# Qualcomm-AI-research/transformer-quantization

Measured on AMD Instinct MI355X. Metric: M elems/sec fake-quant fwd (BERT-base act tensor); achieved HBM GB/s vs peak, higher is better.
Workload: dtype f32; 1 GPU; BERT-base W8A8 per-tensor asym 8-bit activation fake-quant, running-minmax calibrated, fixed-range fwd, hidden [1024,512,768] bf16 per GPU (BASELINE configs[1]); storage_dtype=bf16, parallelism=dp1 (independent shards, no data-path collective)

## Files before the change

transformer-quantization_amd/csrc_py/tq_fastcall.c:

```c
#define PY_SSIZE_T_CLEAN
#include <Python.h>
#include <stdint.h>

typedef int (*fq_fwd_t)(const void*, void*, void*, int, uint64_t, int, const void*, void*);

static int as_u64(PyObject* o, uint64_t* out) {
  if (o == Py_None) { *out = 0; return 0; }
  unsigned long long v = PyLong_AsUnsignedLongLong(o);
  if (v == (unsigned long long)-1 && PyErr_Occurred()) return -1;
  *out = (uint64_t)v;
  return 0;
}

static PyObject* fake_quant_fwd(PyObject* self, PyObject* const* args, Py_ssize_t nargs) {
  (void)self;
  if (nargs != 9) {
    PyErr_SetString(PyExc_TypeError, "fake_quant_fwd(fn, x, y, idx, idx_dtype, n, dtype, q, stream)");
    return NULL;
  }
  uint64_t v[9];
  for (int i = 0; i < 9; ++i)
    if (as_u64(args[i], &v[i])) return NULL;
  if (v[0] == 0) {
    PyErr_SetString(PyExc_ValueError, "fake_quant_fwd: NULL entry point");
    return NULL;
  }
  fq_fwd_t fn = (fq_fwd_t)(uintptr_t)v[0];
  int rc = fn((const void*)(uintptr_t)v[1], (void*)(uintptr_t)v[2], (void*)(uintptr_t)v[3], (int)v[4], v[5], (int)v[6],
              (const void*)(uintptr_t)v[7], (void*)(uintptr_t)v[8]);
  return PyLong_FromLong(rc);
}

typedef int (*calib_tensor_t)(const void*, uint64_t, int, int, const float*, const float*, float*, float*, double, int, int,
                              float, int, float*, float*, uint8_t*, void*, void*, size_t, uint32_t*, void*);

static PyObject* calibrate_tensor(PyObject* self, PyObject* const* args, Py_ssize_t nargs) {
  (void)self;
  if (nargs != 22) {
    PyErr_SetString(PyExc_TypeError, "calibrate_tensor(fn, <the 21 arguments of tq_calibrate_tensor>)");
    return NULL;
  }
  uint64_t v[22];
  double momentum = 0.0, eps = 0.0;
  for (int i = 0; i < 22; ++i) {
    if (i == 9 || i == 12) {
      const double d = PyFloat_AsDouble(args[i]);
      if (d == -1.0 && PyErr_Occurred()) return NULL;
      if (i == 9) momentum = d; else eps = d;
      v[i] = 0;
    } else if (as_u64(args[i], &v[i])) {
      return NULL;
    }
  }
  if (v[0] == 0) {
    PyErr_SetString(PyExc_ValueError, "calibrate_tensor: NULL entry point");
    return NULL;
  }
  calib_tensor_t fn = (calib_tensor_t)(uintptr_t)v[0];
#define P(i) ((void*)(uintptr_t)v[i])
  int rc = fn(P(1), v[2], (int)v[3], (int)v[4], (const float*)P(5), (const float*)P(6), (float*)P(7), (float*)P(8), momentum,
              (int)v[10], (int)v[11], (float)eps, (int)v[13], (float*)P(14), (float*)P(15), (uint8_t*)P(16), P(17), P(18),
              (size_t)v[19], (uint32_t*)P(20), P(21));
#undef P
  return PyLong_FromLong(rc);
}

typedef int (*ptr12_t)(uintptr_t, uintptr_t, uintptr_t, uintptr_t, uintptr_t, uintptr_t, uintptr_t, uintptr_t, uintptr_t,
                       uintptr_t, uintptr_t, uintptr_t);

static PyObject* call_ptrs(PyObject* self, PyObject* const* args, Py_ssize_t nargs) {
  (void)self;
  if (nargs < 1 || nargs > 13) {
    PyErr_SetString(PyExc_TypeError, "call_ptrs(fn, up to 12 integer / pointer arguments)");
    return NULL;
  }
  uint64_t v[13] = {0};
  for (Py_ssize_t i = 0; i < nargs; ++i)
    if (as_u64(args[i], &v[i])) return NULL;
  if (v[0] == 0) {
    PyErr_SetString(PyExc_ValueError, "call_ptrs: NULL entry point");
    return NULL;
  }
  int rc = ((ptr12_t)(uintptr_t)v[0])(v[1], v[2], v[3], v[4], v[5], v[6], v[7], v[8], v[9], v[10], v[11], v[12]);
  return PyLong_FromLong(rc);
}

static PyMethodDef methods[] = {
    {"fake_quant_fwd", (PyCFunction)(void (*)(void))fake_quant_fwd, METH_FASTCALL, "tq_fake_quant_fwd through a raw address"},
    {"calibrate_tensor", (PyCFunction)(void (*)(void))calibrate_tensor, METH_FASTCALL, "tq_calibrate_tensor through a raw address"},
    {"call_ptrs", (PyCFunction)(void (*)(void))call_ptrs, METH_FASTCALL, "int f(uintptr_t...) through a raw address"},
    {NULL, NULL, 0, NULL}};

static struct PyModuleDef moddef = {PyModuleDef_HEAD_INIT, "_tq_fastcall", "fast foreign calls into libtq_hip.so", -1, methods,
                                    NULL, NULL, NULL, NULL};

PyMODINIT_FUNC PyInit__tq_fastcall(void) { return PyModule_Create(&moddef); }
```

transformer-quantization_amd/quantization/_hip.py:

```python
import ctypes as C
import os

import torch

_HERE = os.path.dirname(os.path.abspath(__file__))
LIB_PATH = os.environ.get('TQ_LIB_PATH') or os.path.join(os.path.dirname(_HERE), 'lib', 'libtq_hip.so')

TQ_F32, TQ_BF16, TQ_F16 = 0, 1, 2
IDX_NONE, IDX_F32, IDX_I8, IDX_U8, IDX_I16, IDX_I32, IDX_I8_M128 = range(7)
ACT_NONE, ACT_RELU, ACT_GELU, ACT_TANH = range(4)
EST_CURRENT, EST_ALL, EST_RUNNING = 0, 1, 2
ADA_SIGMOID, ADA_HARD_SIGMOID, ADA_SIGMOID_TEMP = 0, 1, 2

_DTYPES = {torch.float32: TQ_F32, torch.bfloat16: TQ_BF16, torch.float16: TQ_F16}
_IDX_DTYPES = {torch.float32: IDX_F32, torch.int8: IDX_I8, torch.uint8: IDX_U8,
               torch.int16: IDX_I16, torch.int32: IDX_I32}


class TQError(RuntimeError):
    pass


class tq_quantizer(C.Structure):
    _fields_ = [('delta', C.c_void_p), ('zero_float', C.c_void_p), ('signed_flag', C.c_void_p),
# ... 130 lines not shown
    'tq_mse_candidates_grouped': (_int, [_vp, _u64, _u64, _u64, _int, _vp, _u64, _vp, _vp, _sz, _vp]),
    'tq_mse_ordered_workspace_bytes': (_sz, [_u64, _u64, _u64]),
    'tq_mse_candidates_ordered': (_int, [_vp, _u64, _u64, _int, _vp, _u64, _int, _vp, _vp, _vp, _sz, _vp]),
    'tq_xent_candidates': (_int, [_vp, _u64, _u64, _vp, _u64, _vp, _vp]),
    'tq_argmin_select': (_int, [_vp, _u64, _u64, _vp, _vp, _vp, _vp, _vp, _vp]),
    'tq_adaround_fwd': (_int, [_vp, _vp, _vp, _u64, _QP, _int, _int, _f, _vp]),
    'tq_adaround_init_alpha': (_int, [_vp, _vp, _u64, _QP, _int, _f, _vp]),
    'tq_adaround_bwd': (_int, [_vp, _vp, _vp, _vp, _u64, _QP, _int, _f, _vp]),
    'tq_adaround_bwd_adam_sched': (_int, [_vp, _vp, _vp, _vp, _vp, _u64, _QP, _int, _f, _vp, _f, _f, _f, _f, _vp]),
    'tq_adaround_bwd_adam': (_int, [_vp, _vp, _vp, _vp, _vp, _vp, _u64, _QP, _int, _f, _f, _f, _f,
                                    _f, _f, _f, _int, _vp]),
    'tq_adaround_reg': (_int, [_vp, _u64, _int, _f, _f, _f, _vp, _vp, _sz, _vp]),
    'tq_reduce_workspace_bytes': (_sz, [_u64]),
    'tq_recon_loss': (_int, [_vp, _vp, _u64, _u64, _u64, _vp, _vp, _sz, _vp]),
}

_lib = None


def load_library(path=None):
    global _lib
    if _lib is not None and path is None:
        return _lib
    p = path or LIB_PATH
    if not os.path.exists(p):
        raise TQError(
            f'{p} not found: build it with `python transformer-quantization_amd/build.py` '
            '(hipcc --offload-arch=gfx950).  There is no CPU fallback.')
    lib = C.CDLL(p)
    for name, (res, args) in SIGNATURES.items():
        fn = getattr(lib, name)
        fn.restype = res
        fn.argtypes = args
    if lib.tq_abi_version() != ABI_VERSION:
        raise TQError('libtq_hip.so ABI version mismatch: the library says %d, this binding is written for %d -- rebuild '
                      '(python transformer-quantization_amd/build.py)' % (lib.tq_abi_version(), ABI_VERSION))
    if path is None:
        _lib = lib
    return lib


_fastcall_mod, _fastcall_tried = None, False


def fastcall():
    global _fastcall_mod, _fastcall_tried
    if _fastcall_tried:
        return _fastcall_mod
    _fastcall_tried = True
    if os.environ.get('TQ_FASTCALL', '1') == '0':
        return None
    import glob
    import importlib.machinery
    import importlib.util
    for path in sorted(glob.glob(os.path.join(os.path.dirname(LIB_PATH), '_tq_fastcall*.so'))):
        try:
            loader = importlib.machinery.ExtensionFileLoader('_tq_fastcall', path)
            spec = importlib.util.spec_from_loader('_tq_fastcall', loader)
            mod = importlib.util.module_from_spec(spec)
            loader.exec_module(mod)
            _fastcall_mod = mod
            break
        except Exception:
            continue
    return _fastcall_mod


def entry_address(fn):
    return C.cast(fn, C.c_void_p).value


def _check(rc, lib):
    if rc != 0:
        raise TQError(f'libtq_hip: {lib.tq_last_error().decode()} (code {rc})')


def _ptr(t):
    return None if t is None else t.data_ptr()


_raw_stream = getattr(torch._C, '_cuda_getCurrentRawStream', None)


def _stream():
    if _raw_stream is not None:
        return _raw_stream(torch.cuda.current_device())
    return torch.cuda.current_stream().cuda_stream


def _need_device(t, what):
    if not t.is_cuda:
        raise TQError(f'{what}: tensor lives on {t.device}; the fake-quant path only runs on a '
                      'ROCm device (no CPU fallback)')


def _need_f32(what, *tensors):
    for t in tensors:
        if t is not None and t.dtype != torch.float32:
            raise TQError(f'{what}: fp32 tensors required, got {t.dtype} (call .float() on the layer first)')


def _dtype_code(t, what):
    try:
        return _DTYPES[t.dtype]
    except KeyError:
        hint = ' -- float64 (--double) runs the layered quantizer path only' if t.dtype == torch.float64 else ''
        raise TQError(f'{what}: dtype {t.dtype} not supported (fp32 / bf16 / fp16){hint}') from None


def _device_guarded(fn):
    import functools

    _Tensor, _cur = torch.Tensor, torch.cuda.current_device

    @functools.wraps(fn)
    def wrapper(self, *args, **kwargs):
        idx = -1
        for a in args:
            if isinstance(a, _Tensor):
                i = a.get_device()
                if i < 0:
                    continue
                if idx < 0:
                    idx = i
                elif i != idx:
                    raise TQError(f'{fn.__name__}: operands live on different devices (cuda:{idx} and cuda:{i})')
        if idx < 0:
            for a in args:
                if isinstance(a, (tuple, list)):
                    for b in a:
                        if isinstance(b, _Tensor) and b.get_device() >= 0:
                            idx = b.get_device()
                            break
                    if idx >= 0:
                        break
        if idx < 0 or idx == _cur():
            return fn(self, *args, **kwargs)
        with torch.cuda.device(idx):
            return fn(self, *args, **kwargs)
    return wrapper


class HipBackend:

    name = 'hip'

    def __init__(self):
        self.lib = load_library()
        self._ws = {}
        self._qdesc_cache = {}
        self._ws_bytes = {}
        self._counters = {}
        self._calib_tensor_addr = None

    def _workspace(self, device, nbytes):
        key = (device.index, _stream())
        ws = self._ws.get(key)
        if ws is None or ws.numel() < nbytes:
            ws = torch.empty(max(int(nbytes), 1 << 16), dtype=torch.uint8, device=device)
            self._ws[key] = ws
        return ws

    def _calib_ws_bytes(self, n, n_params, inner):
        key = (n, n_params, inner)
        v = self._ws_bytes.get(key)
        if v is None:
            if len(self._ws_bytes) > 4096:
                self._ws_bytes.clear()
            v = self._ws_bytes[key] = self.lib.tq_calibrate_workspace_bytes(n, n_params, inner)
        return v

    def to_device_f32(self, v, like=None):
        if torch.is_tensor(v):
            if v.is_cuda:
                return v if v.dtype == torch.float32 else v.float()
            dev = like.device if (like is not None and like.is_cuda) else torch.device(
                'cuda', torch.cuda.current_device())
            return v.detach().to(device=dev, dtype=torch.float32)
        dev = like.device if (like is not None and like.is_cuda) else torch.device(
            'cuda', torch.cuda.current_device())
        return torch.tensor(v, dtype=torch.float64).float().to(dev)

    def _qdesc(self, delta, zero_float, signed, n_bits, symmetric, log_domain, eps, n_params, inner):
        key = (None if delta is None else delta.data_ptr(), None if zero_float is None else zero_float.data_ptr(),
               None if signed is None else signed.data_ptr(), n_bits, symmetric, log_domain, eps, n_params, inner)
        cache = self._qdesc_cache
        d = cache.get(key)
        if d is None:
            if len(cache) > 8192:
                cache.clear()
            d = cache[key] = tq_quantizer(key[0], key[1], key[2], int(n_bits), int(bool(symmetric)),
                                          int(bool(log_domain)), float(eps), int(n_params), int(inner))
        return d

    @staticmethod
    def _as_f64(t, like):
        if t is None:
            return None
        t = t.detach()
        if t.dtype != torch.float64 or t.device != like.device:
            t = t.to(device=like.device, dtype=torch.float64)
        return t.contiguous()

    def _qdesc_f64(self, delta, zero_float, signed, n_bits, symmetric, log_domain, eps, n_params, inner):
        return tq_quantizer_f64(_ptr(delta), _ptr(zero_float), _ptr(signed), int(n_bits), int(bool(symmetric)),
                                int(bool(log_domain)), 0, float(eps), int(n_params), int(inner))

    def _fake_quant_f64(self, x, delta, zero_float, signed, n_bits, symmetric, log_domain, eps, n_params, inner,
                        want_y, want_idx):
        x = x.contiguous()
        d, z = self._as_f64(delta, x), self._as_f64(zero_float, x)
        y = torch.empty_like(x) if want_y else None
        idx = torch.empty_like(x) if want_idx else None
        q = self._qdesc_f64(d, z, signed, n_bits, symmetric, log_domain, eps, n_params, inner)
        rc = self.lib.tq_fake_quant_fwd_f64(_ptr(x), _ptr(y), _ptr(idx), x.numel(), C.byref(q), _stream())
        _check(rc, self.lib)
        return y, idx

    def fake_quant(self, x, delta, zero_float, signed, n_bits, symmetric, log_domain, eps,
                   n_params, inner, want_y=True, idx_dtype=None):
        _need_device(x, 'fake_quant')
        if x.dtype == torch.float64:
            if idx_dtype not in (None, torch.float32, torch.float64):
                raise TQError('fake_quant: float64 tensors emit float64 indices only')
            return self._fake_quant_f64(x, delta, zero_float, signed, n_bits, symmetric, log_domain, eps, n_params,
                                        inner, want_y, idx_dtype is not None)
        x = x.contiguous()
        y = torch.empty_like(x) if want_y else None
        idx = torch.empty(x.shape, dtype=idx_dtype, device=x.device) if idx_dtype is not None else None
        q = self._qdesc(delta, zero_float, signed, n_bits, symmetric, log_domain, eps, n_params, inner)
        rc = self.lib.tq_fake_quant_fwd(_ptr(x), _ptr(y), _ptr(idx),
                                        _IDX_DTYPES[idx_dtype] if idx_dtype is not None else IDX_NONE,
                                        x.numel(), _dtype_code(x, 'fake_quant'), C.byref(q), _stream())
        _check(rc, self.lib)
        return y, idx

    def fake_quant_multi_plan(self, items):
        arr = (tq_fq_item * max(len(items), 1))()
        ys, keep = [], []
        dtype = items[0][0].dtype if items else torch.float32
        for k, (x, delta, zf, signed, n_bits, symmetric, log_domain, eps, n_params, inner) in enumerate(items):
            _need_device(x, 'fake_quant_multi')
            if x.dtype != dtype:
                raise TQError('fake_quant_multi: all tensors must share one dtype')
            x = x.contiguous()
            y = torch.empty_like(x)
            keep.append((x, delta, zf, signed))
            ys.append(y)
            arr[k].x, arr[k].y, arr[k].n = x.data_ptr(), y.data_ptr(), x.numel()
            arr[k].q = tq_quantizer(_ptr(delta), _ptr(zf), _ptr(signed), int(n_bits), int(bool(symmetric)),
                                    int(bool(log_domain)), float(eps), int(n_params), int(inner))
        return arr, ys, keep, (_dtype_code(items[0][0], 'fake_quant_multi') if items else 0)

    def fake_quant_multi_launch(self, plan):
        arr, ys, _, code = plan
        if ys:
            _check(self.lib.tq_fake_quant_multi_fwd(arr, len(ys), code, _stream()), self.lib)
        return ys

    def fake_quant_multi(self, items):
        return self.fake_quant_multi_launch(self.fake_quant_multi_plan(items)) if items else []

    def fixed_quant_plan(self, delta, zero_float, signed, n_bits, symmetric, log_domain, eps):
        d = self._qdesc(delta, zero_float, signed, n_bits, symmetric, log_domain, eps, 1, 1)
        fc = fastcall()
        if fc is not None:
            return fc.fake_quant_fwd, (entry_address(self.lib.tq_fake_quant_fwd), C.addressof(d)), d
        return self.lib.tq_fake_quant_fwd, C.byref(d), d

    def affine_fake_quant(self, x, w, b, delta, zero_float, signed, n_bits, symmetric, log_domain, eps, want_idx=False):
        _need_device(x, 'affine_fake_quant')
        x = x.contiguous()
        y = torch.empty_like(x)
        idx = torch.empty(x.shape, dtype=torch.int8, device=x.device) if want_idx else None
        q = self._qdesc(delta, zero_float, signed, n_bits, symmetric, log_domain, eps, 1, 1)
        rc = self.lib.tq_affine_fake_quant_fwd(_ptr(x), _ptr(w.detach().float().contiguous()),
                                               _ptr(b.detach().float().contiguous()), _ptr(y), _ptr(idx), x.numel(),
                                               x.shape[-1], _dtype_code(x, 'affine_fake_quant'),
                                               C.byref(q), _stream())
        _check(rc, self.lib)
        return (y, idx) if want_idx else y

    def residual_layernorm_quant(self, dense_out, residual, q_dense, q_sum, ln_weight, ln_bias, ln_eps, q_out,
                                 want_idx=False):
        _need_device(dense_out, 'residual_layernorm_quant')
        a, r = dense_out.contiguous(), residual.contiguous().to(dense_out.dtype)
        y = torch.empty_like(a)
        idx = torch.empty(a.shape, dtype=torch.int8, device=a.device) if want_idx else None
        d = a.shape[-1]
        descs = [None if q is None else self._qdesc(*q, 1, 1) for q in (q_dense, q_sum, q_out)]
        refs = [None if dsc is None else C.byref(dsc) for dsc in descs]
        w32, b32 = ln_weight.detach().float().contiguous(), ln_bias.detach().float().contiguous()
        if ln_eps is None:
            rc = self.lib.tq_residual_nonorm_quant_fwd(
                _ptr(a), _ptr(r), _ptr(y), _ptr(idx), a.numel() // d, d, _dtype_code(a, 'residual_layernorm_quant'),
                refs[0], refs[1], _ptr(w32), _ptr(b32), refs[2], _stream())
        else:
            rc = self.lib.tq_residual_layernorm_quant_fwd(
                _ptr(a), _ptr(r), _ptr(y), _ptr(idx), a.numel() // d, d, _dtype_code(a, 'residual_layernorm_quant'),
                refs[0], refs[1], _ptr(w32), _ptr(b32), float(ln_eps), refs[2], _stream())
        _check(rc, self.lib)
        return (y, idx) if want_idx else y

    def residual_layernorm_quant_axis(self, dense_out, residual, q_dense, q_sum, ln_weight, ln_bias, ln_eps, q_out,
                                      want_idx=False):
        _need_device(dense_out, 'residual_layernorm_quant_axis')
        a, r = dense_out.contiguous(), residual.contiguous().to(dense_out.dtype)
        y = torch.empty_like(a)
        idx = torch.empty(a.shape, dtype=torch.int8, device=a.device) if want_idx else None
        d = a.shape[-1]
        descs = [None if q is None else self._qdesc(*q, 1 if q[0].numel() == 1 else q[0].numel(), 1)
                 for q in (q_dense, q_sum, q_out)]
        refs = [None if dsc is None else C.byref(dsc) for dsc in descs]
        w32, b32 = ln_weight.detach().float().contiguous(), ln_bias.detach().float().contiguous()
        rc = self.lib.tq_residual_layernorm_quant_axis_fwd(
            _ptr(a), _ptr(r), _ptr(y), _ptr(idx), a.numel() // d, d, _dtype_code(a, 'residual_layernorm_quant_axis'),
            refs[0], refs[1], _ptr(w32), _ptr(b32), float(ln_eps), refs[2], _stream())
        _check(rc, self.lib)
        return (y, idx) if want_idx else y

    def embeddings_layernorm_quant(self, word, word_ids, type_tab, type_ids, pos_tab, pos_ids, q_sum1, q_sum2, ln_weight,
                                   ln_bias, ln_eps, q_out, want_idx=False):
        _need_device(word, 'embeddings_layernorm_quant')
        self.raise_deferred()
        _need_f32('embeddings_layernorm_quant', word, type_tab, pos_tab)
        tabs = [t.detach().contiguous() for t in (word, type_tab, pos_tab)]
        ids = [i.reshape(-1).contiguous() for i in (word_ids, type_ids, pos_ids)]
        rows, d = ids[0].numel(), tabs[0].shape[-1]
        if any(i.numel() != rows or i.dtype != torch.int64 for i in ids) or any(t.shape[-1] != d for t in tabs):
            raise TQError('embeddings_layernorm_quant: ids must be int64 of one length, tables of one width')
        y = torch.empty((rows, d), dtype=torch.float32, device=word.device)
        idx = torch.empty((rows, d), dtype=torch.int8, device=word.device) if want_idx else None
        descs = [None if q is None else self._qdesc(*q, 1, 1) for q in (q_sum1, q_sum2, q_out)]
        refs = [None if dsc is None else C.byref(dsc) for dsc in descs]
        w32, b32 = ln_weight.detach().float().contiguous(), ln_bias.detach().float().contiguous()
        rc = self.lib.tq_embeddings_layernorm_quant_fwd(
            _ptr(tabs[0]), tabs[0].shape[0], _ptr(ids[0]), _ptr(tabs[1]), tabs[1].shape[0], _ptr(ids[1]), _ptr(tabs[2]),
            tabs[2].shape[0], _ptr(ids[2]), _ptr(y), _ptr(idx), rows, d, refs[0], refs[1], _ptr(w32), _ptr(b32), float(ln_eps),
            refs[2], self._bad_ids_flag().data_ptr(), _stream())
        _check(rc, self.lib)
        return (y, idx) if want_idx else y

    def _bad_ids_flag(self):
        f = self.__dict__.get('_bad_ids')
        if f is None:
            f = self.__dict__['_bad_ids'] = torch.zeros(1, dtype=torch.int32).pin_memory()
        return f

    def raise_deferred(self, sync=False):
        f = self.__dict__.get('_bad_ids')
        if f is None:
            return
        if sync and not torch.cuda.is_current_stream_capturing():
            torch.cuda.synchronize()
        if int(f[0]) != 0:
            f.zero_()
            raise IndexError('index out of range in self (an embedding id outside its table reached '
                             'tq_embeddings_layernorm_quant_fwd; the rows it produced are NaN)')

    def attention_i8(self, q_idx, k_idx, v_idx, num_heads, mask, denom, q_q, q_k, q_v, q_scores, q_probs, q_ctx,
                     want_idx=False):
        _need_device(q_idx, 'attention_i8')
        B, T, D = q_idx.shape
        rows = lambda t: t.stride(2) == 1 and t.stride(0) == T * t.stride(1) and t.stride(1) % 16 == 0
        if not (rows(q_idx) and rows(k_idx) and rows(v_idx) and k_idx.stride() == q_idx.stride()):
            q_idx, k_idx, v_idx = q_idx.contiguous(), k_idx.contiguous(), v_idx.contiguous()
        ctx = torch.empty((B, T, D), dtype=torch.float32, device=q_idx.device)
        ctx_idx = torch.empty((B, T, D), dtype=torch.int8, device=q_idx.device) if want_idx else None
        descs = [None if q is None else self._qdesc(*q, 1, 1) for q in (q_q, q_k, q_v, q_scores, q_probs, q_ctx)]
        refs = [None if dsc is None else C.byref(dsc) for dsc in descs]
        rc = self.lib.tq_attention_i8_strided_fwd(_ptr(q_idx), _ptr(k_idx), _ptr(v_idx), _ptr(ctx), _ptr(ctx_idx), B, T,
                                                  num_heads, D // num_heads, q_idx.stride(1), v_idx.stride(1), _ptr(mask),
                                                  float(denom), *refs, _stream())
        _check(rc, self.lib)
        return (ctx, ctx_idx) if want_idx else ctx

    def linear_i8_grouped(self, x_idx, w_idx, w_rowsum, bias, x_q, w_delta_rows, w_eps, activation, q_outs,
                          want_y=False, want_idx=True, out_dtype=torch.float32):
        K = x_idx.shape[-1]
        M = x_idx.numel() // K
        N = w_idx.shape[0]
        y = torch.empty(x_idx.shape[:-1] + (N,), dtype=out_dtype, device=x_idx.device) if want_y else None
        y_idx = torch.empty(x_idx.shape[:-1] + (N,), dtype=torch.int8, device=x_idx.device) if want_idx else None
        descs = [self._qdesc(*q, 1, 1) for q in q_outs]
        arr = (C.POINTER(tq_quantizer) * len(descs))(*[C.pointer(d) for d in descs])
        rc = self.lib.tq_linear_i8_grouped_fwd(
            _ptr(x_idx), _ptr(w_idx), _ptr(w_rowsum), _ptr(bias), _ptr(y), _ptr(y_idx), _DTYPES[out_dtype], M, N, K,
            _ptr(x_q[0]), _ptr(x_q[1]), int(x_q[2]), float(x_q[3]), _ptr(w_delta_rows), float(w_eps), int(activation),
            len(descs), C.cast(arr, C.POINTER(_QP)), _stream())
        _check(rc, self.lib)
        return y, y_idx

    def scores_softmax_quant(self, scores, mask, rows_per_mask, denom, q_scores, q_probs):
        _need_device(scores, 'scores_softmax_quant')
        s = scores.contiguous()
        y = torch.empty_like(s)
        cols = s.shape[-1]
        descs = [None if q is None else self._qdesc(*q, 1, 1) for q in (q_scores, q_probs)]
        refs = [None if dsc is None else C.byref(dsc) for dsc in descs]
        rc = self.lib.tq_scores_softmax_quant_fwd(_ptr(s), _ptr(y), s.numel() // cols, cols, _ptr(mask),
                                                  int(rows_per_mask), float(denom), refs[0], refs[1], _stream())
        _check(rc, self.lib)
        return y

    def fake_quant_int8(self, x, delta, zero_float, n_bits, eps):
        _need_device(x, 'fake_quant_int8')
        x = x.contiguous()
        y = torch.empty_like(x)
        idx = torch.empty(x.shape, dtype=torch.int8, device=x.device)
        q = self._qdesc(delta, zero_float, None, n_bits, False, False, eps, 1, 1)
        rc = self.lib.tq_fake_quant_fwd(_ptr(x), _ptr(y), _ptr(idx), IDX_I8_M128, x.numel(),
                                        _dtype_code(x, 'fake_quant_int8'), C.byref(q), _stream())
        _check(rc, self.lib)
        return y, idx

    def quantize_to_int8(self, x, delta, zero_float, signed, n_bits, symmetric, log_domain, eps, n_params,
                         inner, minus_128):
        _need_device(x, 'quantize_to_int8')
        x = x.contiguous()
        idx = torch.empty(x.shape, dtype=torch.int8, device=x.device)
        q = self._qdesc(delta, zero_float, signed, n_bits, symmetric, log_domain, eps, n_params, inner)
        rc = self.lib.tq_fake_quant_fwd(_ptr(x), None, _ptr(idx), IDX_I8_M128 if minus_128 else IDX_I8,
                                        x.numel(), _dtype_code(x, 'quantize_to_int8'), C.byref(q), _stream())
        _check(rc, self.lib)
        return idx

    def rowsum_i8(self, w_idx):
        out = torch.empty(w_idx.shape[0], dtype=torch.int32, device=w_idx.device)
        rc = self.lib.tq_rowsum_i8(_ptr(w_idx), _ptr(out), w_idx.shape[0], w_idx.shape[1], _stream())
        _check(rc, self.lib)
        return out

    STAIR_BINS = 768
    STAIR_BINS_BIG = 1536

    def stair_bins_for(self, M, N):
        big = M % 128 == 0 and N % 128 == 0 and (M // 128) * (N // 128) >= 1024
        return self.STAIR_BINS_BIG if big else self.STAIR_BINS

    def act_stair(self, activation, q_out, n_bins=None):
        n_bins = int(n_bins or self.STAIR_BINS)
        dev = q_out[0].device
        table = torch.empty(self.lib.tq_act_stair_bytes(n_bins), dtype=torch.uint8, device=dev)
        qd = self._qdesc(*q_out, 1, 1)
        rc = self.lib.tq_act_stair_build(int(activation), C.byref(qd), n_bins, table.data_ptr(), table.numel(), _stream())
        _check(rc, self.lib)
        return table, n_bins

    def linear_i8(self, x_idx, w_idx, w_rowsum, bias, x_q, w_delta, w_eps, activation, q_out, out_dtype,
                  want_idx=False, want_y=True, stair=None):
        K = x_idx.shape[-1]
        M = x_idx.numel() // K
        N = w_idx.shape[0]
        shape = x_idx.shape[:-1] + (N,)
        y = torch.empty(shape, dtype=out_dtype, device=x_idx.device) if want_y else None
        y_idx = torch.empty(shape, dtype=torch.int8, device=x_idx.device) if want_idx else None
        qd = None if q_out is None else self._qdesc(*q_out, 1, 1)
        rc = self.lib.tq_linear_i8_stair_fwd(
            _ptr(x_idx), _ptr(w_idx), _ptr(w_rowsum), _ptr(bias), _ptr(y), _ptr(y_idx), _DTYPES[out_dtype], M, N, K,
            _ptr(x_q[0]), _ptr(x_q[1]), int(x_q[2]), float(x_q[3]), _ptr(w_delta), w_delta.numel(),
            float(w_eps), int(activation), None if qd is None else C.byref(qd),
            None if stair is None else stair[0].data_ptr(), 0 if stair is None else int(stair[1]), _stream())
        _check(rc, self.lib)
        return (y, y_idx) if want_idx else y

    SKINNY_MAX_ROWS, SKINNY_MAX_K = 256, 16384

    def linear_i8_skinny(self, x_idx, w_idx, w_rowsum, bias, x_q, w_delta, w_eps, activation, q_out, out_dtype,
                         want_idx=False, want_y=True):
        if x_idx.dim() != 2 or x_idx.dtype != torch.int8 or (x_idx.shape[1] > 1 and x_idx.stride(1) != 1):
            raise TQError('linear_i8_skinny: x_idx must be a 2-D int8 tensor or view whose rows are contiguous')
        M, K = x_idx.shape
        if M > 1 and x_idx.stride(0) < K:
            raise TQError('linear_i8_skinny: rows of x_idx overlap')
        N = w_idx.shape[0]
        y = torch.empty((M, N), dtype=out_dtype, device=x_idx.device) if want_y else None
        y_idx = torch.empty((M, N), dtype=torch.int8, device=x_idx.device) if want_idx else None
        qd = None if q_out is None else self._qdesc(*q_out, 1, 1)
        rc = self.lib.tq_linear_i8_skinny_fwd(
            _ptr(x_idx), x_idx.stride(0) if M > 1 else 0, _ptr(w_idx), _ptr(w_rowsum), _ptr(bias), _ptr(y), _ptr(y_idx),
            _DTYPES[out_dtype], M, N, K, _ptr(x_q[0]), _ptr(x_q[1]), int(x_q[2]), float(x_q[3]), _ptr(w_delta),
            w_delta.numel(), float(w_eps), int(activation), None if qd is None else C.byref(qd), _stream())
        _check(rc, self.lib)
        return (y, y_idx) if want_idx else y

    def cls_table(self, ends, reps):
        t = tq_cls_table()
        t.n_classes = len(ends)
        for c, (e, r) in enumerate(zip(ends, reps)):
            t.end[c], t.rep[c] = int(e), int(r)
        return t

    def cls_stair_bins_for(self, M, N, K, n_classes):
        return self.lib.tq_linear_i8_cls_stair_bins(M, N, K, n_classes) or None

    def linear_i8_cls(self, x_idx, w_idx, cls_rowsum, bias, x_q, cls, w_delta, w_eps, activation, q_out, out_dtype,
                      want_idx=False, want_y=True, stair=None):
        K = x_idx.shape[-1]
        M = x_idx.numel() // K
        N = w_idx.shape[0]
        shape = x_idx.shape[:-1] + (N,)
        y = torch.empty(shape, dtype=out_dtype, device=x_idx.device) if want_y else None
        y_idx = torch.empty(shape, dtype=torch.int8, device=x_idx.device) if want_idx else None
        qd = None if q_out is None else self._qdesc(*q_out, 1, 1)
        rc = self.lib.tq_linear_i8_cls_fwd(
            _ptr(x_idx), _ptr(w_idx), _ptr(cls_rowsum), _ptr(bias), _ptr(y), _ptr(y_idx), _DTYPES[out_dtype], M, N, K,
            _ptr(x_q[0]), _ptr(x_q[1]), x_q[0].numel(), int(x_q[2]), float(x_q[3]), C.byref(cls), _ptr(w_delta),
            w_delta.numel(), float(w_eps), int(activation), None if qd is None else C.byref(qd),
            None if stair is None else stair[0].data_ptr(), 0 if stair is None else int(stair[1]), _stream())
        _check(rc, self.lib)
        return (y, y_idx) if want_idx else y

    def quantize_hilo(self, x, q4):
        _need_device(x, 'quantize_hilo')
        x = x.contiguous()
        hi = torch.empty(x.shape, dtype=torch.int8, device=x.device)
        lo = torch.empty(x.shape, dtype=torch.int8, device=x.device)
        q = self._qdesc(q4[0], q4[1], None, q4[2], False, False, q4[3], 1, 1)
        rc = self.lib.tq_quantize_hilo_fwd(_ptr(x), _ptr(hi), _ptr(lo), x.numel(), _dtype_code(x, 'quantize_hilo'),
                                           C.byref(q), _stream())
        _check(rc, self.lib)
        return hi, lo

    def i16x8_stair_bins_for(self, M, N, K):
        return self.lib.tq_linear_i16x8_stair_bins(M, N, K) or None

    def linear_i16x8(self, x_hi, x_lo, w_idx, w_rowsum, bias, x_q, w_delta, w_eps, activation, q_out, out_dtype,
                     want_idx=False, want_y=True, stair=None):
        K = x_hi.shape[-1]
        M = x_hi.numel() // K
        N = w_idx.shape[0]
        shape = x_hi.shape[:-1] + (N,)
        y = torch.empty(shape, dtype=out_dtype, device=x_hi.device) if want_y else None
        y_idx = torch.empty(shape, dtype=torch.int8, device=x_hi.device) if want_idx else None
        qd = None if q_out is None else self._qdesc(*q_out, 1, 1)
        rc = self.lib.tq_linear_i16x8_fwd(
            _ptr(x_hi), _ptr(x_lo), _ptr(w_idx), _ptr(w_rowsum), _ptr(bias), _ptr(y), _ptr(y_idx), _DTYPES[out_dtype], M, N, K,
            _ptr(x_q[0]), _ptr(x_q[1]), int(x_q[2]), float(x_q[3]), _ptr(w_delta), w_delta.numel(),
            float(w_eps), int(activation), None if qd is None else C.byref(qd),
            None if stair is None else stair[0].data_ptr(), 0 if stair is None else int(stair[1]), _stream())
        _check(rc, self.lib)
        return (y, y_idx) if want_idx else y

    def linear_i8_nonorm(self, x_idx, w_idx, w_rowsum, bias, residual, nn_w, nn_b, x_q, w_delta, w_eps, q_dense, q_sum,
                         q_out, out_dtype, want_idx=False):
        K = x_idx.shape[-1]
        M = x_idx.numel() // K
        N = w_idx.shape[0]
        y = torch.empty(x_idx.shape[:-1] + (N,), dtype=out_dtype, device=x_idx.device)
        y_idx = torch.empty(y.shape, dtype=torch.int8, device=y.device) if want_idx else None
        descs = [None if q is None else self._qdesc(*q, 1, 1) for q in (q_dense, q_sum, q_out)]
        refs = [None if d is None else C.byref(d) for d in descs]
        if residual is not None:
            residual = residual.detach().float().contiguous()
        rc = self.lib.tq_linear_i8_nonorm_fwd(
            _ptr(x_idx), _ptr(w_idx), _ptr(w_rowsum), _ptr(bias), _ptr(residual), _ptr(nn_w.detach().float().contiguous()),
            _ptr(nn_b.detach().float().contiguous()), _ptr(y), _ptr(y_idx), _DTYPES[out_dtype], M, N, K, _ptr(x_q[0]),
            _ptr(x_q[1]), int(x_q[2]), float(x_q[3]), _ptr(w_delta), w_delta.numel(), float(w_eps), refs[0], refs[1],
            refs[2], _stream())
        _check(rc, self.lib)
        return (y, y_idx) if want_idx else y

    def linear_i8_nonorm_grouped(self, x_idx, w_idx, w_rowsum, bias, nn_w, nn_b, x_q, w_delta_rows, w_eps, q_dense, q_out,
                                 out_dtype, want_idx=False, n_groups=2):
        K = x_idx.shape[-1]
        M = x_idx.numel() // K
        N = w_idx.shape[0]
        G = int(n_groups)
        y = torch.empty((G,) + tuple(x_idx.shape[:-1]) + (N // G,), dtype=out_dtype, device=x_idx.device)
        y_idx = torch.empty(y.shape, dtype=torch.int8, device=y.device) if want_idx else None

        def arr(qs):
            if qs is None:
                return None, None
            descs = [self._qdesc(*q, 1, 1) for q in qs]
            return descs, C.cast((C.POINTER(tq_quantizer) * G)(*[C.pointer(d) for d in descs]), C.POINTER(_QP))
        keep_d, a_d = arr(q_dense)
        keep_o, a_o = arr(q_out)
        rc = self.lib.tq_linear_i8_nonorm_grouped_fwd(
            _ptr(x_idx), _ptr(w_idx), _ptr(w_rowsum), _ptr(bias), _ptr(nn_w), _ptr(nn_b), _ptr(y), _ptr(y_idx),
            _DTYPES[out_dtype], M, N, K, _ptr(x_q[0]), _ptr(x_q[1]), int(x_q[2]), float(x_q[3]), _ptr(w_delta_rows),
            float(w_eps), G, a_d, a_o, _stream())
        _check(rc, self.lib)
        ys = [y[g] for g in range(G)]
        return (ys, [y_idx[g] for g in range(G)]) if want_idx else ys

    def ffn_chain_i8_nonorm(self, x_idx, x_q, residual, stages, out_dtype, want_idx=False):
        K1 = x_idx.shape[-1]
        M = x_idx.numel() // K1
        N1, N2 = stages[0]['w1_idx'].shape[0], stages[0]['w2_idx'].shape[0]
        y = torch.empty(x_idx.shape[:-1] + (N2,), dtype=out_dtype, device=x_idx.device)
        y_idx = torch.empty(y.shape, dtype=torch.int8, device=y.device) if want_idx else None
        keep = []
        arr = (tq_ffn_stage * len(stages))()
        for a, g in zip(arr, stages):
            def qp(q):
                if q is None:
                    return None
                d = self._qdesc(*q, 1, 1)
                keep.append(d)
                return C.pointer(d)

            def f32(t):
                t = t.detach().float().contiguous()
                keep.append(t)
                return t.data_ptr()
            a.w1_idx, a.w1_rowsum, a.bias1 = _ptr(g['w1_idx']), _ptr(g['w1_rowsum']), _ptr(g['bias1'])
            a.w1_delta, a.w1_n_params, a.w1_eps = _ptr(g['w1_delta']), g['w1_delta'].numel(), float(g['w1_eps'])
            a.q_mid = qp(g['q_mid'])
            a.w2_idx, a.w2_rowsum, a.bias2 = _ptr(g['w2_idx']), _ptr(g['w2_rowsum']), _ptr(g['bias2'])
# ... 558 lines not shown
```

Before: 1.584 million M elems/s.

## Add cached C launch records for fused-route entry points to cut ctypes overhead

Adds C fastcall stubs for the linear, attention, layernorm and embeddings entry points, plus a LaunchRecord vectorcall object. The record converts the fixed arguments of a call site once and fills in only the per-call pointers at launch. The Python backend caches these records by shape, parameter pointers and descriptor ids, which removes the per-call ctypes marshalling cost. The metric here is the fake-quant fwd path, which these routes do not touch. Caching on data_ptr and id() risks stale records if memory is reused.

```diff
diff --git a/transformer-quantization_amd/csrc_py/tq_fastcall.c b/transformer-quantization_amd/csrc_py/tq_fastcall.c
--- a/transformer-quantization_amd/csrc_py/tq_fastcall.c
+++ b/transformer-quantization_amd/csrc_py/tq_fastcall.c
@@ -1,6 +1,8 @@
 #define PY_SSIZE_T_CLEAN
 #include <Python.h>
+#include <stddef.h>
 #include <stdint.h>
+#include <string.h>
 
 typedef int (*fq_fwd_t)(const void*, void*, void*, int, uint64_t, int, const void*, void*);
 
@@ -85,13 +87,265 @@
   return PyLong_FromLong(rc);
 }
 
+enum { E_LINEAR_STAIR, E_LINEAR_GROUPED, E_ATTENTION, E_ATTENTION_STRIDED, E_TAIL_LN, E_EMBEDDINGS_LN, E_COUNT };
+#define MAX_ARGS 22
+
+static const struct entry_sig {
+  const char* name;
+  int nargs;
+  uint32_t floats;
+} ENTRIES[E_COUNT] = {
+    {"linear_i8_stair_fwd", 22, (1u << 13) | (1u << 16)},
+    {"linear_i8_grouped_fwd", 20, (1u << 13) | (1u << 15)},
+    {"attention_i8_fwd", 19, 1u << 11},
+    {"attention_i8_strided_fwd", 20, 1u << 12},
+    {"residual_layernorm_quant_fwd", 14, 1u << 11},
+    {"embeddings_layernorm_quant_fwd", 21, 1u << 17},
+};
+
+typedef const void* cp;
+typedef int (*linear_stair_t)(cp, cp, cp, cp, void*, void*, int, uint64_t, uint64_t, uint64_t, cp, cp, int, float, cp, uint64_t,
+                              float, int, cp, cp, uint32_t, void*);
+typedef int (*linear_grouped_t)(cp, cp, cp, cp, void*, void*, int, uint64_t, uint64_t, uint64_t, cp, cp, int, float, cp, float,
+                                int, uint64_t, cp, void*);
+typedef int (*attention_t)(cp, cp, cp, void*, void*, uint64_t, uint64_t, uint64_t, uint64_t, uint64_t, cp, float, cp, cp, cp, cp,
+                           cp, cp, void*);
+typedef int (*attention_strided_t)(cp, cp, cp, void*, void*, uint64_t, uint64_t, uint64_t, uint64_t, uint64_t, uint64_t, cp, float,
+                                   cp, cp, cp, cp, cp, cp, void*);
+typedef int (*tail_ln_t)(cp, cp, void*, void*, uint64_t, uint64_t, int, cp, cp, cp, cp, float, cp, void*);
+typedef int (*embeddings_ln_t)(cp, uint64_t, cp, cp, uint64_t, cp, cp, uint64_t, cp, void*, void*, uint64_t, uint64_t, cp, cp, cp,
+                               cp, float, cp, void*, void*);
+
+static int dispatch(int entry, uintptr_t fn, const uint64_t* v, const float* f) {
+#define P(i) ((void*)(uintptr_t)v[i])
+#define I(i) ((int)v[i])
+  switch (entry) {
+    case E_LINEAR_STAIR:
+      return ((linear_stair_t)fn)(P(0), P(1), P(2), P(3), P(4), P(5), I(6), v[7], v[8], v[9], P(10), P(11), I(12), f[13], P(14),
+                                  v[15], f[16], I(17), P(18), P(19), (uint32_t)v[20], P(21));
+    case E_LINEAR_GROUPED:
+      return ((linear_grouped_t)fn)(P(0), P(1), P(2), P(3), P(4), P(5), I(6), v[7], v[8], v[9], P(10), P(11), I(12), f[13], P(14),
+                                    f[15], I(16), v[17], P(18), P(19));
+    case E_ATTENTION:
+      return ((attention_t)fn)(P(0), P(1), P(2), P(3), P(4), v[5], v[6], v[7], v[8], v[9], P(10), f[11], P(12), P(13), P(14),
+                               P(15), P(16), P(17), P(18));
+    case E_ATTENTION_STRIDED:
+      return ((attention_strided_t)fn)(P(0), P(1), P(2), P(3), P(4), v[5], v[6], v[7], v[8], v[9], v[10], P(11), f[12], P(13),
+                                       P(14), P(15), P(16), P(17), P(18), P(19));
+    case E_TAIL_LN:
+      return ((tail_ln_t)fn)(P(0), P(1), P(2), P(3), v[4], v[5], I(6), P(7), P(8), P(9), P(10), f[11], P(12), P(13));
+    default:
+      return ((embeddings_ln_t)fn)(P(0), v[1], P(2), P(3), v[4], P(5), P(6), v[7], P(8), P(9), P(10), v[11], v[12], P(13), P(14),
+                                   P(15), P(16), f[17], P(18), P(19), P(20));
+  }
+#undef P
+#undef I
+}
+
+static int convert(int e, PyObject* const* args, uint32_t skip, uint64_t* v, float* f) {
+  for (int i = 0; i < ENTRIES[e].nargs; ++i) {
+    if (skip >> i & 1u) continue;
+    if (ENTRIES[e].floats >> i & 1u) {
+      const double d = PyFloat_AsDouble(args[i]);
+      if (d == -1.0 && PyErr_Occurred()) return -1;
+      f[i] = (float)d;
+    } else if (as_u64(args[i], &v[i])) {
+      return -1;
+    }
+  }
+  return 0;
+}
+
+static int entry_point(const char* name, PyObject* o, uintptr_t* fn) {
+  uint64_t a;
+  if (as_u64(o, &a)) return -1;
+  if (a == 0) {
+    PyErr_Format(PyExc_ValueError, "%s: NULL entry point", name);
+    return -1;
+  }
+  *fn = (uintptr_t)a;
+  return 0;
+}
+
+static PyObject* stub_call(int e, PyObject* const* args, Py_ssize_t nargs) {
+  if (nargs != ENTRIES[e].nargs + 1) {
+    PyErr_Format(PyExc_TypeError, "%s(fn, <the %d arguments of tq_%s>)", ENTRIES[e].name, ENTRIES[e].nargs, ENTRIES[e].name);
+    return NULL;
+  }
+  uint64_t v[MAX_ARGS] = {0};
+  float f[MAX_ARGS] = {0};
+  uintptr_t fn;
+  if (convert(e, args + 1, 0, v, f) || entry_point(ENTRIES[e].name, args[0], &fn)) return NULL;
+  return PyLong_FromLong(dispatch(e, fn, v, f));
+}
+
+#define STUB(fname, e) \
+  static PyObject* fname(PyObject* self, PyObject* const* args, Py_ssize_t nargs) { (void)self; return stub_call(e, args, nargs); }
+STUB(linear_i8_stair_fwd, E_LINEAR_STAIR)
+STUB(linear_i8_grouped_fwd, E_LINEAR_GROUPED)
+STUB(attention_i8_fwd, E_ATTENTION)
+STUB(attention_i8_strided_fwd, E_ATTENTION_STRIDED)
+STUB(residual_layernorm_quant_fwd, E_TAIL_LN)
+STUB(embeddings_layernorm_quant_fwd, E_EMBEDDINGS_LN)
+#undef STUB
+
+#define MAX_DYN 8
+
+typedef struct {
+  PyObject_HEAD
+  vectorcallfunc vectorcall;
+  int entry, ndyn;
+  uintptr_t fn;
+  uint8_t dyn[MAX_DYN];
+  uint64_t v[MAX_ARGS];
+  float f[MAX_ARGS];
+  PyObject* keep;
+} Record;
+
+static PyObject* record_call(PyObject* self, PyObject* const* args, size_t nargsf, PyObject* kwnames) {
+  Record* r = (Record*)self;
+  if (PyVectorcall_NARGS(nargsf) != r->ndyn || (kwnames && PyTuple_GET_SIZE(kwnames))) {
+    PyErr_Format(PyExc_TypeError, "launch record of %s takes %d positional arguments", ENTRIES[r->entry].name, r->ndyn);
+    return NULL;
+  }
+  uint64_t v[MAX_ARGS];
+  memcpy(v, r->v, sizeof v);
+  for (int i = 0; i < r->ndyn; ++i)
+    if (as_u64(args[i], &v[r->dyn[i]])) return NULL;
+  return PyLong_FromLong(dispatch(r->entry, r->fn, v, r->f));
+}
+
+static void record_dealloc(PyObject* self) {
+  Py_XDECREF(((Record*)self)->keep);
+  Py_TYPE(self)->tp_free(self);
+}
+
+static PyObject* record_args(PyObject* self, void* closure) {
+  (void)closure;
+  Record* r = (Record*)self;
+  const int n = ENTRIES[r->entry].nargs;
+  PyObject* t = PyTuple_New(n);
+  if (!t) return NULL;
+  for (int i = 0; i < n; ++i) {
+    int is_dyn = 0;
+    for (int k = 0; k < r->ndyn; ++k) is_dyn |= r->dyn[k] == i;
+    PyObject* o;
+    if (is_dyn) {
+      o = Py_None;
+      Py_INCREF(o);
+    } else if (ENTRIES[r->entry].floats >> i & 1u) {
+      o = PyFloat_FromDouble(r->f[i]);
+    } else {
+      o = PyLong_FromUnsignedLongLong(r->v[i]);
+    }
+    if (!o) {
+      Py_DECREF(t);
+      return NULL;
+    }
+    PyTuple_SET_ITEM(t, i, o);
+  }
+  return t;
+}
+
+static PyObject* record_entry(PyObject* self, void* closure) {
+  (void)closure;
+  return PyUnicode_FromString(ENTRIES[((Record*)self)->entry].name);
+}
+
+static PyGetSetDef record_getset[] = {{"args", record_args, NULL, "arguments held (None at the per-call slots)", NULL},
+                                      {"entry", record_entry, NULL, "name of the entry point", NULL},
+                                      {NULL, NULL, NULL, NULL, NULL}};
+
+static PyTypeObject RecordType = {
+    PyVarObject_HEAD_INIT(NULL, 0).tp_name = "_tq_fastcall.LaunchRecord",
+    .tp_basicsize = sizeof(Record),
+    .tp_dealloc = record_dealloc,
+    .tp_vectorcall_offset = offsetof(Record, vectorcall),
+    .tp_call = PyVectorcall_Call,
+    .tp_flags = Py_TPFLAGS_DEFAULT | Py_TPFLAGS_HAVE_VECTORCALL,
+    .tp_getset = record_getset,
+    .tp_doc = "the unchanging arguments of one call site of a fused-route entry point, converted once",
+};
+
+static PyObject* launch_record(PyObject* self, PyObject* const* args, Py_ssize_t nargs) {
+  (void)self;
+  if (nargs != 5 || !PyUnicode_Check(args[0]) || !PyTuple_Check(args[2]) || !PyTuple_Check(args[3])) {
+    PyErr_SetString(PyExc_TypeError, "launch_record(entry: str, fn: int, args: tuple, dyn: tuple, keep)");
+    return NULL;
+  }
+  const char* name = PyUnicode_AsUTF8(args[0]);
+  if (!name) return NULL;
+  int e = 0;
+  while (e < E_COUNT && strcmp(name, ENTRIES[e].name)) ++e;
+  if (e == E_COUNT) {
+    PyErr_Format(PyExc_ValueError, "launch_record: unknown entry point %s", name);
+    return NULL;
+  }
+  const Py_ssize_t ndyn = PyTuple_GET_SIZE(args[3]);
+  if (PyTuple_GET_SIZE(args[2]) != ENTRIES[e].nargs || ndyn > MAX_DYN) {
+    PyErr_Format(PyExc_TypeError, "launch_record: %s takes %d arguments, at most %d of them per call", name, ENTRIES[e].nargs,
+                 MAX_DYN);
+    return NULL;
+  }
+  uint8_t dyn[MAX_DYN];
+  uint32_t skip = 0;
+  for (Py_ssize_t i = 0; i < ndyn; ++i) {
+    const long s = PyLong_AsLong(PyTuple_GET_ITEM(args[3], i));
+    if (s == -1 && PyErr_Occurred()) return NULL;
+    if (s < 0 || s >= ENTRIES[e].nargs || (ENTRIES[e].floats >> s & 1u) || (skip >> s & 1u)) {
+      PyErr_Format(PyExc_ValueError, "launch_record: %ld is not a per-call slot of %s (in range, not a float, named once)", s, name);
+      return NULL;
+    }
+    dyn[i] = (uint8_t)s;
+    skip |= 1u << s;
+  }
+  uintptr_t fn;
+  if (entry_point(name, args[1], &fn)) return NULL;
+  Record* r = PyObject_New(Record, &RecordType);
+  if (!r) return NULL;
+  r->vectorcall = record_call;
+  r->entry = e;
+  r->ndyn = (int)ndyn;
+  r->fn = fn;
+  r->keep = NULL;
+  memset(r->v, 0, sizeof r->v);
+  memset(r->f, 0, sizeof r->f);
+  memcpy(r->dyn, dyn, sizeof dyn);
+  if (convert(e, &PyTuple_GET_ITEM(args[2], 0), skip, r->v, r->f)) {
+    Py_DECREF(r);
+    return NULL;
+  }
+  Py_INCREF(args[4]);
+  r->keep = args[4];
+  return (PyObject*)r;
+}
+
+#define FASTCALL(f, doc) {#f, (PyCFunction)(void (*)(void))f, METH_FASTCALL, doc}
 static PyMethodDef methods[] = {
-    {"fake_quant_fwd", (PyCFunction)(void (*)(void))fake_quant_fwd, METH_FASTCALL, "tq_fake_quant_fwd through a raw address"},
-    {"calibrate_tensor", (PyCFunction)(void (*)(void))calibrate_tensor, METH_FASTCALL, "tq_calibrate_tensor through a raw address"},
-    {"call_ptrs", (PyCFunction)(void (*)(void))call_ptrs, METH_FASTCALL, "int f(uintptr_t...) through a raw address"},
+    FASTCALL(fake_quant_fwd, "tq_fake_quant_fwd through a raw address"),
+    FASTCALL(calibrate_tensor, "tq_calibrate_tensor through a raw address"),
+    FASTCALL(call_ptrs, "int f(uintptr_t...) through a raw address"),
+    FASTCALL(linear_i8_stair_fwd, "tq_linear_i8_stair_fwd through a raw address"),
+    FASTCALL(linear_i8_grouped_fwd, "tq_linear_i8_grouped_fwd through a raw address"),
+    FASTCALL(attention_i8_fwd, "tq_attention_i8_fwd through a raw address"),
+    FASTCALL(attention_i8_strided_fwd, "tq_attention_i8_strided_fwd through a raw address"),
+    FASTCALL(residual_layernorm_quant_fwd, "tq_residual_layernorm_quant_fwd through a raw address"),
+    FASTCALL(embeddings_layernorm_quant_fwd, "tq_embeddings_layernorm_quant_fwd through a raw address"),
+    FASTCALL(launch_record, "the unchanging arguments of a call site, converted once -> a callable record"),
     {NULL, NULL, 0, NULL}};
 
 static struct PyModuleDef moddef = {PyModuleDef_HEAD_INIT, "_tq_fastcall", "fast foreign calls into libtq_hip.so", -1, methods,
                                     NULL, NULL, NULL, NULL};
 
-PyMODINIT_FUNC PyInit__tq_fastcall(void) { return PyModule_Create(&moddef); }
+PyMODINIT_FUNC PyInit__tq_fastcall(void) {
+  if (PyType_Ready(&RecordType) < 0) return NULL;
+  PyObject* m = PyModule_Create(&moddef);
+  if (!m) return NULL;
+  Py_INCREF(&RecordType);
+  if (PyModule_AddObject(m, "LaunchRecord", (PyObject*)&RecordType) < 0) {
+    Py_DECREF(&RecordType);
+    Py_DECREF(m);
+    return NULL;
+  }
+  return m;
+}
diff --git a/transformer-quantization_amd/quantization/_hip.py b/transformer-quantization_amd/quantization/_hip.py
--- a/transformer-quantization_amd/quantization/_hip.py
+++ b/transformer-quantization_amd/quantization/_hip.py
@@ -306,6 +306,8 @@
         self._ws_bytes = {}
         self._counters = {}
         self._calib_tensor_addr = None
+        self._records = {}
+        self._entry_addrs = {}
 
     def _workspace(self, device, nbytes):
         key = (device.index, _stream())
@@ -346,6 +348,20 @@
             d = cache[key] = tq_quantizer(key[0], key[1], key[2], int(n_bits), int(bool(symmetric)),
                                           int(bool(log_domain)), float(eps), int(n_params), int(inner))
         return d
+
+    RECORDS_MAX = 4096
+
+    def _entry(self, entry):
+        a = self._entry_addrs.get(entry)
+        if a is None:
+            a = self._entry_addrs[entry] = entry_address(getattr(self.lib, 'tq_' + entry))
+        return a
+
+    def _new_record(self, fc, key, args, dyn, keep):
+        if len(self._records) >= self.RECORDS_MAX:
+            self._records.clear()
+        rec = self._records[key] = fc.launch_record(key[0], self._entry(key[0]), args, dyn, keep)
+        return rec
 
     @staticmethod
     def _as_f64(t, like):
@@ -438,11 +454,27 @@
     def residual_layernorm_quant(self, dense_out, residual, q_dense, q_sum, ln_weight, ln_bias, ln_eps, q_out,
                                  want_idx=False):
         _need_device(dense_out, 'residual_layernorm_quant')
-        a, r = dense_out.contiguous(), residual.contiguous().to(dense_out.dtype)
+        a, r = dense_out.contiguous(), residual.contiguous()
+        if r.dtype != a.dtype:
+            r = r.to(a.dtype)
         y = torch.empty_like(a)
-        idx = torch.empty(a.shape, dtype=torch.int8, device=a.device) if want_idx else None
+        idx = a.new_empty(a.shape, dtype=torch.int8) if want_idx else None
         d = a.shape[-1]
         descs = [None if q is None else self._qdesc(*q, 1, 1) for q in (q_dense, q_sum, q_out)]
+        fc = fastcall()
+        if fc is not None and ln_eps is not None:
+            rows, code = a.numel() // d, _dtype_code(a, 'residual_layernorm_quant')
+            key = ('residual_layernorm_quant_fwd', rows, d, code, id(descs[0]), id(descs[1]), id(descs[2]),
+                   ln_weight.data_ptr(), ln_weight._version, ln_weight.dtype, ln_weight.stride(),
+                   ln_bias.data_ptr(), ln_bias._version, ln_bias.dtype, ln_bias.stride(), float(ln_eps))
+            rec = self._records.get(key)
+            if rec is None:
+                w32, b32 = ln_weight.detach().float().contiguous(), ln_bias.detach().float().contiguous()
+                qa = [0 if dsc is None else C.addressof(dsc) for dsc in descs]
+                rec = self._new_record(fc, key, (0, 0, 0, 0, rows, d, code, qa[0], qa[1], w32.data_ptr(), b32.data_ptr(),
+                                                 key[-1], qa[2], 0), (0, 1, 2, 3, 13), (descs, ln_weight, ln_bias, w32, b32))
+            _check(rec(a.data_ptr(), r.data_ptr(), y.data_ptr(), _ptr(idx), _stream()), self.lib)
+            return (y, idx) if want_idx else y
         refs = [None if dsc is None else C.byref(dsc) for dsc in descs]
         w32, b32 = ln_weight.detach().float().contiguous(), ln_bias.detach().float().contiguous()
         if ln_eps is None:
@@ -486,8 +518,18 @@
         y = torch.empty((rows, d), dtype=torch.float32, device=word.device)
         idx = torch.empty((rows, d), dtype=torch.int8, device=word.device) if want_idx else None
         descs = [None if q is None else self._qdesc(*q, 1, 1) for q in (q_sum1, q_sum2, q_out)]
+        w32, b32 = ln_weight.detach().float().contiguous(), ln_bias.detach().float().contiguous()
+        fc = fastcall()
+        if fc is not None:
+            qa = [0 if dsc is None else C.addressof(dsc) for dsc in descs]
+            rc = fc.embeddings_layernorm_quant_fwd(
+                self._entry('embeddings_layernorm_quant_fwd'), tabs[0].data_ptr(), tabs[0].shape[0], ids[0].data_ptr(),
+                tabs[1].data_ptr(), tabs[1].shape[0], ids[1].data_ptr(), tabs[2].data_ptr(), tabs[2].shape[0],
+                ids[2].data_ptr(), y.data_ptr(), _ptr(idx), rows, d, qa[0], qa[1], w32.data_ptr(), b32.data_ptr(),
+                float(ln_eps), qa[2], self._bad_ids_flag().data_ptr(), _stream())
+            _check(rc, self.lib)
+            return (y, idx) if want_idx else y
         refs = [None if dsc is None else C.byref(dsc) for dsc in descs]
-        w32, b32 = ln_weight.detach().float().contiguous(), ln_bias.detach().float().contiguous()
         rc = self.lib.tq_embeddings_layernorm_quant_fwd(
             _ptr(tabs[0]), tabs[0].shape[0], _ptr(ids[0]), _ptr(tabs[1]), tabs[1].shape[0], _ptr(ids[1]), _ptr(tabs[2]),
             tabs[2].shape[0], _ptr(ids[2]), _ptr(y), _ptr(idx), rows, d, refs[0], refs[1], _ptr(w32), _ptr(b32), float(ln_eps),
@@ -516,15 +558,29 @@
                      want_idx=False):
         _need_device(q_idx, 'attention_i8')
         B, T, D = q_idx.shape
-        rows = lambda t: t.stride(2) == 1 and t.stride(0) == T * t.stride(1) and t.stride(1) % 16 == 0
-        if not (rows(q_idx) and rows(k_idx) and rows(v_idx) and k_idx.stride() == q_idx.stride()):
+        sq, sk, sv = q_idx.stride(), k_idx.stride(), v_idx.stride()
+        if not (sk == sq and sq[2] == 1 and sq[0] == T * sq[1] and sq[1] % 16 == 0
+                and sv[2] == 1 and sv[0] == T * sv[1] and sv[1] % 16 == 0):
             q_idx, k_idx, v_idx = q_idx.contiguous(), k_idx.contiguous(), v_idx.contiguous()
-        ctx = torch.empty((B, T, D), dtype=torch.float32, device=q_idx.device)
-        ctx_idx = torch.empty((B, T, D), dtype=torch.int8, device=q_idx.device) if want_idx else None
+            sq, sv = q_idx.stride(), v_idx.stride()
+        ctx = q_idx.new_empty((B, T, D), dtype=torch.float32)
+        ctx_idx = q_idx.new_empty((B, T, D), dtype=torch.int8) if want_idx else None
         descs = [None if q is None else self._qdesc(*q, 1, 1) for q in (q_q, q_k, q_v, q_scores, q_probs, q_ctx)]
+        fc = fastcall()
+        if fc is not None:
+            key = ('attention_i8_strided_fwd', B, T, num_heads, D, sq[1], sv[1], float(denom),
+                   id(descs[0]), id(descs[1]), id(descs[2]), id(descs[3]), id(descs[4]), id(descs[5]))
+            rec = self._records.get(key)
+            if rec is None:
+                qa = [0 if dsc is None else C.addressof(dsc) for dsc in descs]
+                rec = self._new_record(fc, key, (0, 0, 0, 0, 0, B, T, num_heads, D // num_heads, key[5], key[6], 0, key[7],
+                                                 *qa, 0), (0, 1, 2, 3, 4, 11, 19), descs)
+            _check(rec(q_idx.data_ptr(), k_idx.data_ptr(), v_idx.data_ptr(), ctx.data_ptr(), _ptr(ctx_idx), _ptr(mask),
+                       _stream()), self.lib)
+            return (ctx, ctx_idx) if want_idx else ctx
         refs = [None if dsc is None else C.byref(dsc) for dsc in descs]
         rc = self.lib.tq_attention_i8_strided_fwd(_ptr(q_idx), _ptr(k_idx), _ptr(v_idx), _ptr(ctx), _ptr(ctx_idx), B, T,
-                                                  num_heads, D // num_heads, q_idx.stride(1), v_idx.stride(1), _ptr(mask),
+                                                  num_heads, D // num_heads, sq[1], sv[1], _ptr(mask),
                                                   float(denom), *refs, _stream())
         _check(rc, self.lib)
         return (ctx, ctx_idx) if want_idx else ctx
@@ -534,9 +590,25 @@
         K = x_idx.shape[-1]
         M = x_idx.numel() // K
         N = w_idx.shape[0]
-        y = torch.empty(x_idx.shape[:-1] + (N,), dtype=out_dtype, device=x_idx.device) if want_y else None
-        y_idx = torch.empty(x_idx.shape[:-1] + (N,), dtype=torch.int8, device=x_idx.device) if want_idx else None
+        shape = x_idx.shape[:-1] + (N,)
+        y = x_idx.new_empty(shape, dtype=out_dtype) if want_y else None
+        y_idx = x_idx.new_empty(shape, dtype=torch.int8) if want_idx else None
         descs = [self._qdesc(*q, 1, 1) for q in q_outs]
+        fc = fastcall()
+        if fc is not None:
+            key = ('linear_i8_grouped_fwd', w_idx.data_ptr(), _ptr(w_rowsum), None if bias is None else bias.data_ptr(),
+                   out_dtype, M, N, K, x_q[0].data_ptr(), None if x_q[1] is None else x_q[1].data_ptr(), int(x_q[2]),
+                   float(x_q[3]), _ptr(w_delta_rows), float(w_eps), int(activation),
+                   tuple([id(d) for d in descs]))
+            rec = self._records.get(key)
+            if rec is None:
+                arr = (C.c_void_p * len(descs))(*[C.addressof(d) for d in descs])
+                rec = self._new_record(fc, key, (0,) + key[1:4] + (0, 0, _DTYPES[out_dtype]) + key[5:15]
+                                       + (len(descs), C.addressof(arr), 0), (0, 4, 5, 19), (descs, arr))
+            rc = rec(x_idx.data_ptr(), y.data_ptr() if want_y else 0, y_idx.data_ptr() if want_idx else 0, _stream())
+            if rc != 0:
+                _check(rc, self.lib)
+            return y, y_idx
         arr = (C.POINTER(tq_quantizer) * len(descs))(*[C.pointer(d) for d in descs])
         rc = self.lib.tq_linear_i8_grouped_fwd(
             _ptr(x_idx), _ptr(w_idx), _ptr(w_rowsum), _ptr(bias), _ptr(y), _ptr(y_idx), _DTYPES[out_dtype], M, N, K,
@@ -607,9 +679,23 @@
         M = x_idx.numel() // K
         N = w_idx.shape[0]
         shape = x_idx.shape[:-1] + (N,)
-        y = torch.empty(shape, dtype=out_dtype, device=x_idx.device) if want_y else None
-        y_idx = torch.empty(shape, dtype=torch.int8, device=x_idx.device) if want_idx else None
+        y = x_idx.new_empty(shape, dtype=out_dtype) if want_y else None
+        y_idx = x_idx.new_empty(shape, dtype=torch.int8) if want_idx else None
         qd = None if q_out is None else self._qdesc(*q_out, 1, 1)
+        fc = fastcall()
+        if fc is not None:
+            key = ('linear_i8_stair_fwd', w_idx.data_ptr(), _ptr(w_rowsum), None if bias is None else bias.data_ptr(),
+                   out_dtype, M, N, K, x_q[0].data_ptr(), None if x_q[1] is None else x_q[1].data_ptr(), int(x_q[2]),
+                   float(x_q[3]), w_delta.data_ptr(), w_delta.numel(), float(w_eps),
+                   int(activation), id(qd), None if stair is None else stair[0].data_ptr(), 0 if stair is None else int(stair[1]))
+            rec = self._records.get(key)
+            if rec is None:
+                rec = self._new_record(fc, key, (0,) + key[1:4] + (0, 0, _DTYPES[out_dtype]) + key[5:16]
+                                       + (0 if qd is None else C.addressof(qd),) + key[17:19] + (0,), (0, 4, 5, 21), qd)
+            rc = rec(x_idx.data_ptr(), y.data_ptr() if want_y else 0, y_idx.data_ptr() if want_idx else 0, _stream())
+            if rc != 0:
+                _check(rc, self.lib)
+            return (y, y_idx) if want_idx else y
         rc = self.lib.tq_linear_i8_stair_fwd(
             _ptr(x_idx), _ptr(w_idx), _ptr(w_rowsum), _ptr(bias), _ptr(y), _ptr(y_idx), _DTYPES[out_dtype], M, N, K,
             _ptr(x_q[0]), _ptr(x_q[1]), int(x_q[2]), float(x_q[3]), _ptr(w_delta), w_delta.numel(),
```

New measurement: 1.549 million M elems/s. 0.978x the previous value.
